# oneapi-src/ishmem

Hardware: AMD Instinct MI355X
Metric: GiB/s device-resident float32 sum-reduce at 1/2/4/8 PEs vs HBM+xGMI roofline (higher is better)
Workload: dtype f32; 1 GPU; float32 sum-reduce, 1024 MiB per PE, 1 PE(s), symmetric-heap device buffers; nreduce=268435456, bytes_per_pe=1073741824, pes=1, parallelism=1 PE self-reduce

## Files before the change

include/ishmem_capi.h:

```cpp
#ifndef ISHMEM_AMD_CAPI_H
#define ISHMEM_AMD_CAPI_H

#include <stddef.h>
#include <stdint.h>

#ifdef __cplusplus
extern "C" {
#endif

typedef enum {
    ISHMEMI_OP_AND = 0,
    ISHMEMI_OP_OR = 1,
    ISHMEMI_OP_XOR = 2,
    ISHMEMI_OP_MAX = 3,
    ISHMEMI_OP_MIN = 4,
    ISHMEMI_OP_SUM = 5,
    ISHMEMI_OP_PROD = 6,
    ISHMEMI_OP_COUNT = 7
} ishmemi_c_op_t;

typedef enum {
    ISHMEMI_DT_INT8 = 0,
    ISHMEMI_DT_INT16 = 1,
    ISHMEMI_DT_INT32 = 2,
// ... 198 lines not shown
    ISHMEMI_C_PATH_PHASED = 4,
    ISHMEMI_C_PATH_PERSISTENT = 5,
    ISHMEMI_C_PATH_ELEM = 6,
    ISHMEMI_C_PATH_STAGED = 7,
    ISHMEMI_C_PATH_COUNT = 8
} ishmemi_c_path_t;
const char *ishmemi_c_last_error(void);
int ishmemi_c_set_param(const char *name, long long value);
long long ishmemi_c_get_param(const char *name);
int ishmemi_c_phase_times(float *ms5);
int ishmemi_c_error_count(void);
size_t ishmemi_c_dtype_size(int dtype);
int ishmemi_c_op_dtype_valid(int op, int dtype);
int ishmemi_c_chunk_bounds(uint64_t nitems, int npes, int c, uint64_t *begin, uint64_t *end);
int ishmemi_c_path_limits(int npes, int colocated, long long *ll_limit, long long *fold_limit);
int ishmemi_c_bootstrap_selftest(int pe, int npes, const char *key, int value, int *out);
const char *ishmemi_c_version(void);

#ifdef __cplusplus
}
#endif

#endif
```

ishmem_amd/__init__.py:

```python
from __future__ import annotations

import ctypes
import sys

from ._lib import LIB_PATH, load

_L = load()

OPS = {"and": 0, "or": 1, "xor": 2, "max": 3, "min": 4, "sum": 5, "prod": 6}
DTYPES = {"int8": 0, "int16": 1, "int32": 2, "int64": 3, "uint8": 4, "uint16": 5,
          "uint32": 6, "uint64": 7, "float": 8, "double": 9,
          "half": 16, "bfloat16": 17}
ISHMEM_TEAM_INVALID = -1
ISHMEM_TEAM_WORLD = 0
ISHMEM_TEAM_SHARED = 1
ISHMEMX_TEAM_NODE = 2

TYPENAMES = {
    "char": "int8", "schar": "int8", "short": "int16", "int": "int32", "long": "int64",
    "longlong": "int64", "ptrdiff": "int64", "uchar": "uint8", "ushort": "uint16",
    "uint": "uint32", "ulong": "uint64", "ulonglong": "uint64", "int8": "int8",
    "int16": "int16", "int32": "int32", "int64": "int64", "uint8": "uint8", "uint16": "uint16",
    "uint32": "uint32", "uint64": "uint64", "size": "uint64", "float": "float", "double": "double",
}
# ... 178 lines not shown
    return int(_L.ishmemi_c_get_param(name.encode()))


PATH_NAMES = ("none", "single", "granule", "fold", "phased", "persistent", "elem", "staged")


def last_path() -> str:
    return PATH_NAMES[get_param("last_path")]


def path_limits(npes: int, colocated: bool) -> tuple[int, int]:
    ll, fold = ctypes.c_longlong(0), ctypes.c_longlong(0)
    if _L.ishmemi_c_path_limits(npes, int(bool(colocated)), ctypes.byref(ll), ctypes.byref(fold)):
        raise ValueError(f"path_limits: {last_error()}")
    return ll.value, fold.value


def reduce(op: str, dtype: str, dest: int, source: int, nreduce: int, team: int = ISHMEM_TEAM_WORLD) -> int:
    return _L.ishmemi_c_reduce(team, OPS[op], DTYPES[dtype], dest, source, nreduce)


def _event_handle(e) -> int | None:
    return getattr(e, "h", e) or None


def reduce_on_stream(op: str, dtype: str, dest: int, source: int, nreduce: int, ret: int | None,
                     stream: int, team: int = ISHMEM_TEAM_WORLD, deps=(), done=None) -> int:
    if deps or done is not None:
        hs = [_event_handle(e) for e in deps]
        arr = (ctypes.c_void_p * len(hs))(*hs) if hs else None
# ... 550 lines not shown
```

ishmem_amd/_lib.py:

```python
from __future__ import annotations

import ctypes
import os
from pathlib import Path

LIB_PATH = Path(__file__).resolve().parent / "libishmem_amd.so"
_VARIANT = os.environ.get("ISHMEM_AMD_LIB")

_vp, _i, _sz, _ll, _u64 = ctypes.c_void_p, ctypes.c_int, ctypes.c_size_t, ctypes.c_longlong, ctypes.c_uint64
_pd = ctypes.c_ssize_t
PROTOTYPES = [
    ("ishmemi_c_init", _i, []),
    ("ishmemi_c_init_pe", _i, [_i, _i, _i, ctypes.c_char_p]),
    ("ishmemi_c_launch_info", _i, [ctypes.POINTER(_i), ctypes.POINTER(_i), ctypes.POINTER(_i), ctypes.c_char_p, _sz,
                                   ctypes.c_char_p, _sz]),
    ("ishmemi_c_finalize", _i, []),
    ("ishmemi_c_initialized", _i, []),
    ("ishmemi_c_my_pe", _i, []),
    ("ishmemi_c_n_pes", _i, []),
    ("ishmemi_c_device", _i, []),
    ("ishmemi_c_init_thread", _i, [_i, ctypes.POINTER(_i)]),
    ("ishmemi_c_query_thread", _i, [ctypes.POINTER(_i)]),
    ("ishmemi_c_malloc", _vp, [_sz]),
    ("ishmemi_c_align", _vp, [_sz, _sz]),
# ... 63 lines not shown
    ("ishmemi_c_scan", _i, [_i, _i, _i, _vp, _vp, _sz]),
    ("ishmemi_c_scan_on_stream", _i, [_i, _i, _i, _vp, _vp, _sz, _vp, _vp]),
    ("ishmemi_c_broadcast", _i, [_i, _vp, _vp, _sz, _i]),
    ("ishmemi_c_broadcast_on_stream", _i, [_i, _vp, _vp, _sz, _i, _vp, _vp]),
    ("ishmemi_c_device_ctx", _vp, []),
    ("ishmemi_c_register_device_ctx_slot", _i, [_vp]),
    ("ishmemi_c_last_error", ctypes.c_char_p, []),
    ("ishmemi_c_set_param", _i, [ctypes.c_char_p, _ll]),
    ("ishmemi_c_get_param", _ll, [ctypes.c_char_p]),
    ("ishmemi_c_phase_times", _i, [ctypes.POINTER(ctypes.c_float)]),
    ("ishmemi_c_error_count", _i, []),
    ("ishmemi_c_dtype_size", _sz, [_i]),
    ("ishmemi_c_op_dtype_valid", _i, [_i, _i]),
    ("ishmemi_c_chunk_bounds", _i, [_u64, _i, _i, ctypes.POINTER(_u64), ctypes.POINTER(_u64)]),
    ("ishmemi_c_path_limits", _i, [_i, _i, ctypes.POINTER(_ll), ctypes.POINTER(_ll)]),
    ("ishmemi_c_bootstrap_selftest", _i, [_i, _i, ctypes.c_char_p, _i, ctypes.POINTER(_i)]),
    ("ishmemi_c_version", ctypes.c_char_p, []),
]

_lib = None


def load(build_if_missing: bool = True) -> ctypes.CDLL:
    global _lib
    if _lib is not None:
        return _lib
    if _VARIANT:
        lib = ctypes.CDLL(str(Path(_VARIANT).resolve()), mode=ctypes.RTLD_GLOBAL)
        for name, res, args in PROTOTYPES:
            fn = getattr(lib, name)
# ... 36 lines not shown
```

ishmem_amd/csrc/kernels.h:

```cpp
#pragma once
#include <hip/hip_runtime.h>
#include <stddef.h>
#include <stdint.h>

#include "types.h"

namespace ishmemi {

constexpr int kMaxPes = 16;
constexpr int kMaxBlocks = 1024;
constexpr int kPhases = 4;
constexpr int kPhaseStart = 0, kPhaseMid = 1, kPhaseEnd = 2, kPhaseSync = 3;
constexpr size_t kFlagWordsPerTeam = (size_t) kPhases * kMaxBlocks * kMaxPes;
constexpr size_t kTeamFlagBytes = kFlagWordsPerTeam * 4 + 256;
constexpr int kBlock = 256;
constexpr int kUnroll = 4;
constexpr int kFaninBlock = 64;
constexpr int kFaninMaxGrid = (int) ((1ull << 31) / kFaninBlock);

constexpr int kEpWords = 16;
constexpr int kLineWords = 16;
constexpr int kEpReplicas = 64;
constexpr int kEpRepLine = 1, kEpShardLine = kEpRepLine + kEpReplicas, kEpShards = 8;
constexpr int kEpTopLine = kEpShardLine + kEpShards;
// ... 113 lines not shown
#endif
constexpr int kRsRealignBlock = ISHMEMI_RS_REALIGN_BLOCK;
#ifndef ISHMEMI_REALIGN_PEEL
#define ISHMEMI_REALIGN_PEEL 256
#endif
constexpr uint64_t kRealignPeel = ISHMEMI_REALIGN_PEEL;

struct FaninArgs {
    const char *src[kMaxFanin];
    char *dst;
    uint64_t head, nitems, tail;
    int nsrc;
    int realign;
    uint32_t shift[kMaxFanin];
    uint64_t total;
};

struct PhaseArgs {
    const char *src[kMaxPes];
    const char *dstp[kMaxPes];
    char *dst;
    uint64_t head, nitems, tail;
    uint64_t items_per_chunk;
    uint32_t elem;
    int p, me;
    int peer_nt;
    uint32_t shift;
    uint64_t total;
    int whole;
    int xcd_group;
// ... 121 lines not shown
```

ishmem_amd/csrc/kernels_impl.h:

```cpp
#pragma once
#include <algorithm>
#include <map>
#include <mutex>
#include <type_traits>

#include "kernels.h"

namespace ishmemi {
namespace {

constexpr int kSysCoherent = 17;
constexpr int kNonTemporal = 2;
constexpr uint64_t kTile = (uint64_t) kBlock * kUnroll;
#ifndef ISHMEMI_AR_OCC
#define ISHMEMI_AR_OCC 4
#endif


template <typename T>
struct alignas(16) Vec {
    T e[16 / sizeof(T)];
};

template <typename T>
// ... 711 lines not shown

template <typename I>
__device__ __forceinline__ I nt_load(const I *p)
{
    if constexpr (sizeof(I) == 16) return __builtin_bit_cast(I, __builtin_nontemporal_load((const u32x4 *) p));
    else if constexpr (is_fp16_v<I>) return I{__builtin_nontemporal_load((const uint16_t *) p)};
    else return __builtin_nontemporal_load(p);
}

template <typename T, int OP, bool VEC, int NS>
__global__ __launch_bounds__(kFaninBlock) void fanin_kernel(FaninArgs a)
{
    using Item = std::conditional_t<VEC, Vec<T>, T>;
    constexpr uint64_t IB = sizeof(Item);
    const uint64_t head_bytes = VEC ? a.head * sizeof(T) : 0;
    const uint64_t stride = (uint64_t) gridDim.x * kFaninBlock;
    for (uint64_t i = (uint64_t) blockIdx.x * kFaninBlock + threadIdx.x; i < a.nitems; i += stride) {
        const uint64_t off = head_bytes + i * IB;
        Item acc;
        if constexpr (NS == 1) {
            acc = nt_load((const Item *) (a.src[0] + off));
        } else if constexpr (NS == 2 && VEC) {
            const uint64_t wo = off - (uint64_t) threadIdx.x * IB;
            const uint32_t lo = (uint32_t) (threadIdx.x * IB);
            const Item x0 = bload<Item>(make_rsrc(uniform_ptr(a.src[0] + wo)), lo);
            asm volatile("s_waitcnt vmcnt(0)" ::: "memory");
            const Item x1 = bload<Item>(make_rsrc(uniform_ptr(a.src[1] + wo)), lo);
            acc = op1<T, OP>(x0, x1);
        } else if constexpr (NS == 2) {
            const Item x0 = nt_load((const Item *) (a.src[0] + off));
            const Item x1 = nt_load((const Item *) (a.src[1] + off));
            acc = op1<T, OP>(x0, x1);
// ... 76 lines not shown
#pragma unroll
    for (int j = 0; j < NS; ++j) realign_issue<kNonTemporal>(a.src[j], a.shift[j], a.total, wo, edge[j], A[j], B[j]);
    __syncthreads();
    Vec<T> acc = __builtin_bit_cast(Vec<T>, realign_finish(edge[0], A[0], B[0], a.shift[0]));
    if constexpr (NS == 2)
        acc = op1<T, OP>(acc, __builtin_bit_cast(Vec<T>, realign_finish(edge[1], A[1], B[1], a.shift[1])));
    if (i0 + tid < a.nitems) wt_store(make_rsrc(uniform_ptr(a.dst + wo)), tid * 16u, acc);
}

template <typename T, int OP, int NS>
__global__ __launch_bounds__(kRealignBlock) void fanin_realign_kernel(FaninArgs a)
{
    static_assert(NS == 1 || NS == 2, "realigned fan-in: 1 or 2 sources");
    __shared__ u32x4 edge[NS][kRealignWaves + 1];
    const uint32_t tid = threadIdx.x;
    const uint64_t stride = (uint64_t) gridDim.x * kRealignBlock;
    const uint64_t first = (uint64_t) blockIdx.x * kRealignBlock;
    if (stride >= a.nitems) {
        if (first < a.nitems) fanin_realign_block<T, OP, NS>(a, edge, first);
    } else {
        for (uint64_t i0 = first; i0 < a.nitems; i0 += stride) {
            fanin_realign_block<T, OP, NS>(a, edge, i0);
            __syncthreads();
        }
    }
    if (blockIdx.x == 0) {
        const uint64_t tail_off = a.head + a.nitems * (16 / sizeof(T));
        for (int pass = 0; pass < 2; ++pass) {
            const uint64_t cnt = pass == 0 ? a.head : a.tail;
            for (uint64_t t = tid; t < cnt; t += kRealignBlock) {
                const uint64_t e = pass == 0 ? t : tail_off + t;
                T acc = ((const T *) a.src[0])[e];
                if constexpr (NS == 2) acc = op1<T, OP>(acc, ((const T *) a.src[1])[e]);
                ((T *) a.dst)[e] = acc;
            }
        }
    }
// ... 619 lines not shown
```

ishmem_amd/csrc/runtime.cpp:

```cpp
#include <hip/hip_runtime.h>
#include <stdio.h>
#include <stdlib.h>
#include <string.h>
#include <strings.h>
#include <stdint.h>
#include <errno.h>
#include <sys/prctl.h>
#include <unistd.h>

#include <algorithm>
#include <chrono>
#include <limits>
#include <map>
#include <mutex>
#include <string>
#include <vector>

#include "bootstrap.h"
#include "kernels.h"
#include "types.h"

namespace ishmemi {
namespace {

// ... 152 lines not shown
    return s && *s && (strcmp(s, "0") == 0 || strcasecmp(s, "false") == 0);
}
bool env_flag_true(const char *name)
{
    const char *s = getenv(name);
    return s && *s && !env_flag_false(name);
}

void warn_unknown_env()
{
    static const char *const known[] = {
        "DEBUG", "ENABLE_VERBOSE_PRINT", "STACK_PRINT_LIMIT", "ENABLE_GPU_IPC", "ENABLE_GPU_IPC_PIDFD",
        "SYMMETRIC_SIZE", "ENABLE_ACCESSIBLE_HOST_HEAP", "NBI_COUNT", "MWAIT_BURST", "SHMEM_LIB_NAME",
        "MPI_LIB_NAME", "PMI_LIB_NAME", "TEAMS_MAX", "TEAM_SHARED_ONLY_SELF", "RUNTIME", "RUNTIME_USE_OSHMPI", "ROOT",
        "PE", "NPES", "DEVICE", "BOOTSTRAP_KEY", "TIMEOUT_MS", "MAX_BLOCKS", "WAIT_SLOTS", "LL_MAX_BYTES",
        "ONESHOT_P2_MAX_BYTES", "PHASED_MIN_BYTES", "PHASED_PEER_NT", "STAGING_SIZE", "STAGING_SLOTS",
        "STAGED_COPY_KERNEL", "STREAM_ORDER", "FLAGS_KIND", "EP_UNCACHED", "BARRIER_KIND", "XGMI_LL_MAX_BYTES",
        "XGMI_FOLD_MAX_BYTES", "PUT_SIGNAL_FUSED_MAX_BYTES", "TEST_FLAGS_UNAVAILABLE", "TEST_PCI_BUS",
        "AMD_LIB", "OFFLOAD_ARCH", "BENCH_SAME_DEVICE", "BENCH_EMULATE_SHARE1", "BENCH_SETUP_WATCHDOG_S"};
    for (char **e = ::environ; e && *e; ++e) {
        if (strncmp(*e, "ISHMEM_", 7) != 0) continue;
        const char *name = *e + 7, *eq = strchr(name, '=');
        const size_t len = eq ? (size_t) (eq - name) : strlen(name);
        bool ok = false;
        for (const char *k : known) ok = ok || (strlen(k) == len && strncmp(k, name, len) == 0);
        if (!ok) fprintf(stderr, "[ishmem_amd] WARN: Environment variable 'ISHMEM_%.*s' is not a supported variable\n", (int) len, name);
    }
}

long long wait_slots_floor() { return std::max<long long>(1, env_ll("GPU_MAX_HW_QUEUES", 4)); }

// ... 7 lines not shown

struct TeamMem {
    uint32_t *flags[kMaxPes] = {};
    uint64_t *ring[kMaxPes] = {};
    int pool_idx = -1;
    char *fold_scratch = nullptr;
    size_t fold_scratch_bytes = 0;
};

struct PoolBlock {
    uint32_t *ptr = nullptr;
    hipIpcMemHandle_t handle{};
    bool in_use = false;
};

constexpr long long kPhasedOff = std::numeric_limits<long long>::max();
constexpr long long kPhasedDefault = 4ll << 20;

struct PeRecord {
    int32_t pe, pid, device, flags_kind;
    int32_t flags_kind_requested;
    char pci_bus[32];
    uint64_t heap_size;
    int64_t max_blocks, ll_max_bytes, oneshot_p2, phased_min;
    uint64_t staging_bytes;
    int64_t staging_slots;
    int64_t xgmi_ll_max, xgmi_fold_max;
    hipIpcMemHandle_t heap_handle;
    hipIpcMemHandle_t flags_handle;
};
// ... 50 lines not shown
    hipStream_t last_stream = nullptr;
    bool last_stream_set = false;
    bool stream_order = false;
    long long oneshot_p2 = 32ll << 20;
    long long phased_min = kPhasedDefault;
    hipEvent_t order_ev = nullptr;
    hipEvent_t staging_ev = nullptr;
    bool staging_used = false;
    int staging_slots = kStagingSlotsDefault;
    int staged_copy_kernel = 0;
    bool test_flags_unavailable = false;
    int phased_peer_nt = 0;
    int ar_shifted = 1;
    int rs_xcd = 1;
    int last_path = ISHMEMI_C_PATH_NONE;
    int direct_p2 = 1;
    int direct_max_pes = 4;
    int direct_inplace = 1;
    long long xgmi_ll_max = -1, xgmi_fold_max = -1;
    double xgmi_link_bps = 76.8e9;
    hipEvent_t ev_in[kMaxStagingSlots] = {}, ev_red[kMaxStagingSlots] = {}, ev_out[kMaxStagingSlots] = {};

    Team teams[kMaxTeams];
    int max_blocks = kMaxBlocks;
    long long ll_max_bytes = (long long) kLLDefaultBytes;
    long long timeout_ms = 60000;
    int debug = 0;
    int error_count = 0;
    uint64_t *trace = nullptr;
    bool phase_events = false, phase_recorded = false;
// ... 265 lines not shown
    const uintptr_t d = (uintptr_t) dst;
    bool ok = !pl.vec && nsrc >= 1 && nsrc <= 2 && n * es >= kRealignMinBytes && d % es == 0;
    for (int j = 0; ok && j < nsrc; ++j) ok = (uintptr_t) srcs[j] % es == 0;
    if (!ok) return;
    const uint64_t h = std::min<uint64_t>(n, ((kRealignPeel - d % kRealignPeel) % kRealignPeel) / es);
    f.head = h;
    f.nitems = (n - h) * es / 16;
    f.tail = n - h - f.nitems * (16 / es);
    for (int j = 0; j < nsrc; ++j) f.shift[j] = (uint32_t) (((uintptr_t) srcs[j] + h * es) % 16);
    f.total = n * es;
    f.realign = 1;
    pl.grid = (int) std::max<uint64_t>(1, std::min<uint64_t>((f.nitems + kRealignBlock - 1) / kRealignBlock,
                                                             (uint64_t) kRealignMaxGrid));
}

int launch_copy(void *dst, const void *src, size_t bytes, hipStream_t st)
{
    if (bytes == 0 || dst == src) return 0;
    FaninArgs f{};
    f.src[0] = (const char *) src;
    f.dst = (char *) dst;
    f.nsrc = 1;
    const void *srcs[1] = {src};
    Plan pl;
    plan_fanin(f, pl, dst, srcs, 1, bytes, 1);
    HIP_TRY(launch_fanin(ISHMEMI_OP_OR, ISHMEMI_DT_UINT8, pl.vec, f, pl.grid, st));
    return 0;
}

constexpr double kHopUs = 1.0;
constexpr long long kUnlimited = std::numeric_limits<long long>::max();
struct Line {
    double a_us, b_us_per_byte;
};
Line model_ll(int p, double L) { return {4.5 + 0.5 * (p - 2) + 1 * kHopUs, 2e6 / L}; }
Line model_fold(int p, double L) { return {9.0 + 0.75 * (p - 2) + 2 * kHopUs, 1e6 / L}; }
Line model_rsag(int p, double L) { return {9.5 + 2.5 * (p - 2) + 3 * kHopUs, 2e6 / (p * L)}; }

long long crossover(const Line &f, const Line &g)
{
// ... 240 lines not shown
        if (mark(0)) return 1;
        if (team_barrier(a, st)) return 1;
        if (mark(1)) return 1;
        HIP_TRY(launch_rs_phase(op, dt, ph, st));
        if (mark(2)) return 1;
        if (!direct) {
            if (team_barrier(a, st)) return 1;
            if (mark(3)) return 1;
            HIP_TRY(launch_ag_phase(ph, st));
        } else if (mark(3)) {
            return 1;
        }
        if (mark(4)) return 1;
        if (team_barrier(a, st)) return 1;
        if (mark(5)) return 1;
        if (inplace_fold && launch_copy(dst, scratch, nb, st)) return 1;
        s.phase_recorded = s.phase_recorded || ev;
        return 0;
    }
    if (t.size == 2 && (long long) nb <= lim.oneshot && disjoint) {
        a.oneshot = 1;
        a.items_per_chunk = pl.nitems;
        a.seg_items = seg_items(pl.nitems);
        pl.grid = (int) std::max<uint64_t>(
            1, std::min<uint64_t>(nsegs(pl.nitems, a.seg_items), (uint64_t) s.max_blocks));
    }
    s.last_path = ISHMEMI_C_PATH_PERSISTENT;
    HIP_TRY(launch_allreduce(op, dt, pl.vec, a, pl.grid, st));
    return 0;
}

// ... 75 lines not shown
            HIP_TRY(hipEventCreateWithFlags(&s.ev_in[i], hipEventDisableTiming));
            HIP_TRY(hipEventCreateWithFlags(&s.ev_red[i], hipEventDisableTiming));
            HIP_TRY(hipEventCreateWithFlags(&s.ev_out[i], hipEventDisableTiming));
        }
    }
    if (staging_acquire(s, st)) return 1;
    HIP_TRY(hipEventRecord(s.ev_red[0], st));
    HIP_TRY(hipStreamWaitEvent(s.copy_in, s.ev_red[0], 0));
    bool used[kMaxStagingSlots] = {};
    for (size_t off = 0, k = 0; off < n; off += chunk, ++k) {
        const int sl = (int) (k % (size_t) nslots);
        char *buf = s.staging + (size_t) sl * slot_bytes;
        const size_t m = std::min(chunk, n - off);
        if (used[sl]) HIP_TRY(hipStreamWaitEvent(s.copy_in, s.ev_out[sl], 0));
        if (src_dev) {
            if (launch_copy(buf, src_dev + off * es, m * es, s.copy_in)) return 1;
        } else {
            HIP_TRY(hipMemcpyAsync(buf, (const char *) src + off * es, m * es, hipMemcpyDefault, s.copy_in));
        }
        HIP_TRY(hipEventRecord(s.ev_in[sl], s.copy_in));
        HIP_TRY(hipStreamWaitEvent(st, s.ev_in[sl], 0));
        if (s.teams[team].size > 1) {
            const bool ll = ll_eligible(s, s.teams[team], buf, buf, m * es);
            if (ll ? reduce_ll(s, team, op, dt, buf, buf, m * es, ret, st)
                   : reduce_heap(s, team, op, dt, buf, buf, m, ret, st))
                return 1;
        }
        HIP_TRY(hipEventRecord(s.ev_red[sl], st));
        HIP_TRY(hipStreamWaitEvent(s.copy_out, s.ev_red[sl], 0));
        if (dst_dev) {
            if (launch_copy(dst_dev + off * es, buf, m * es, s.copy_out)) return 1;
        } else {
            HIP_TRY(hipMemcpyAsync((char *) dst + off * es, buf, m * es, hipMemcpyDefault, s.copy_out));
        }
        HIP_TRY(hipEventRecord(s.ev_out[sl], s.copy_out));
        used[sl] = true;
    }
    for (int sl = 0; sl < nslots; ++sl)
        if (used[sl]) HIP_TRY(hipStreamWaitEvent(st, s.ev_out[sl], 0));
    return staging_release(s, st);
}

int team_sync_locked(State &s, int team, hipStream_t st, int *ret);

template <typename A>
int fill_team_sync_args(State &s, int team, A &a, std::string &why)
// ... 74 lines not shown
        if (collect_launch(s, team, dst, s.staging, segb, ret, st, segoff)) return 1;
    }
    s.last_path = ISHMEMI_C_PATH_STAGED;
    return staging_release(s, st);
}

int collect_on_stream_impl(int team, void *dst, const void *src, size_t nbytes, int *ret, hipStream_t st)
{
    State &s = S();
    std::lock_guard<std::mutex> lk(s.mu);
    if (team_call(s, "collect", team)) return 1;
    Team &t = s.teams[team];
    if (ret) HIP_TRY(hipMemsetAsync(ret, 0, sizeof(int), st));
    if (t.size == 1) {
        s.last_path = ISHMEMI_C_PATH_SINGLE;
        if (nbytes && dst != src && launch_copy(dst, src, nbytes, st)) return 1;
        return mark_stream(s, st);
    }
    if (!in_heap(s, dst)) return fail("collect: dest must be symmetric-heap memory");
    if (!in_heap(s, src)) return fail("collect: source must be symmetric-heap memory");
    if (order_stream(s, st)) return 1;
    CollectArgs a;
    memset(&a, 0, sizeof(a));
    std::string why;
    if (fill_team_sync_args(s, team, a, why)) return fail("collect: " + why);
    char *slot = s.count_slots + (size_t) team * 64;
    for (int j = 0; j < t.size; ++j) {
        const int gpe = t.start + j * t.stride;
        a.src[j] = translate(s, src, gpe);
        a.count_at[j] = (const uint64_t *) translate(s, slot, gpe);
        if (!a.src[j] || !a.count_at[j]) return fail("collect: buffer not mapped for PE " + std::to_string(gpe));
// ... 8 lines not shown
    s.last_path = ISHMEMI_C_PATH_PERSISTENT;
    HIP_TRY(launch_collect_dyn(a, grid, st));
    return mark_stream(s, st);
}

int fcollect_impl(int team, void *dst, const void *src, size_t nbytes, int *ret, hipStream_t st,
                  bool blocking, int staged = -1)
{
    State &s = S();
    std::lock_guard<std::mutex> lk(s.mu);
    if (team_call(s, "fcollect", team)) return 1;
    Team &t = s.teams[team];
    if (ret) HIP_TRY(hipMemsetAsync(ret, 0, sizeof(int), st));
    if (t.size == 1) {
        s.last_path = ISHMEMI_C_PATH_SINGLE;
        if (nbytes && dst != src && launch_copy(dst, src, nbytes, st)) return 1;
    } else {
        if (staged < 0 && !device_writable(s, dst)) return fail("fcollect: dest must be heap, device or pinned host memory");
        uint64_t nb[kMaxPes];
        for (int j = 0; j < t.size; ++j) nb[j] = nbytes;
        if (staged < 0) staged = in_heap(s, src) ? 0 : 1;
        if (nbytes == 0) {
            s.last_path = ISHMEMI_C_PATH_NONE;
            if (team_sync_locked(s, team, st, ret)) return 1;
        } else if (!staged && ll_eligible(s, t, dst, src, nbytes) && 2 * nbytes <= ll_capacity(t.size)) {
            s.last_path = ISHMEMI_C_PATH_GRANULE;
            if (reduce_ll(s, team, ISHMEMI_OP_OR, ISHMEMI_DT_UINT8, dst, src, nbytes, ret, st, kLLCollect)) return 1;
        } else if (staged) {
            if (order_stream(s, st) || collect_staged(s, team, (char *) dst, (const char *) src, nb, ret, st)) return 1;
        } else if (collect_launch(s, team, dst, src, nb, ret, st)) {
            return 1;
// ... 54 lines not shown
int alltoall_impl(int team, void *dst, const void *src, size_t nbytes, int *ret, hipStream_t st, bool blocking,
                  bool checked)
{
    State &s = S();
    std::lock_guard<std::mutex> lk(s.mu);
    if (team_call(s, "alltoall", team)) return 1;
    Team &t = s.teams[team];
    if (nbytes > 0 && (!dst || !src)) return fail("alltoall: null buffer");
    if (t.size > 1 && nbytes > 0 && !checked) {
        const uint64_t e = alltoall_arg_errors(s, t, dst, src, nbytes);
        if (e) return fail(alltoall_arg_message(e));
    }
    if (ret) HIP_TRY(hipMemsetAsync(ret, 0, sizeof(int), st));
    if (t.size == 1) {
        s.last_path = ISHMEMI_C_PATH_SINGLE;
        if (nbytes && dst != src && launch_copy(dst, src, nbytes, st)) return 1;
    } else if (nbytes == 0) {
        s.last_path = ISHMEMI_C_PATH_NONE;
        if (team_sync_locked(s, team, st, ret)) return 1;
    } else if (ll_eligible(s, t, dst, src, nbytes) && 2 * nbytes <= ll_capacity(t.size)) {
        s.last_path = ISHMEMI_C_PATH_GRANULE;
        if (reduce_ll(s, team, ISHMEMI_OP_OR, ISHMEMI_DT_UINT8, dst, src, nbytes, ret, st, kLLAlltoall)) return 1;
    } else {
        uint64_t nb[kMaxPes], off[kMaxPes];
        const char *srcs[kMaxPes];
        for (int j = 0; j < t.size; ++j) {
            const char *pj = translate(s, src, t.start + j * t.stride);
            if (!pj) return fail("alltoall: source not mapped for PE " + std::to_string(t.start + j * t.stride));
            srcs[j] = pj + (uint64_t) t.my_idx * nbytes;
            off[j] = (uint64_t) j * nbytes;
            nb[j] = nbytes;
// ... 78 lines not shown
{
    State &s = S();
    std::lock_guard<std::mutex> lk(s.mu);
    if (team_call(s, "reduce_scatter", team)) return 1;
    Team &t = s.teams[team];
    if (!op_dtype_valid(op, dt)) return fail("reduce_scatter: invalid (op, dtype) pair");
    if (n > 0 && (!dst || !src)) return fail("reduce_scatter: null buffer");
    if (n > 0 && !checked) {
        const uint64_t e = reduce_scatter_arg_errors(s, t, op, dt, dst, src, n);
        if (e) return fail(reduce_scatter_arg_message(e));
    }
    const size_t B = n * dtype_size(dt);
    if (ret) HIP_TRY(hipMemsetAsync(ret, 0, sizeof(int), st));
    if (t.size == 1) {
        s.last_path = ISHMEMI_C_PATH_SINGLE;
        if (B && launch_copy(device_view(s, dst), src, B, st)) return 1;
    } else if (n == 0) {
        s.last_path = ISHMEMI_C_PATH_NONE;
        if (team_sync_locked(s, team, st, ret)) return 1;
    } else if (ll_eligible(s, t, dst, src, B) && B <= ll_capacity(t.size)) {
        s.last_path = ISHMEMI_C_PATH_GRANULE;
        if (reduce_ll(s, team, op, dt, device_view(s, dst), src, B, ret, st, kLLReduceScatter)) return 1;
    } else if (reduce_scatter_heap(s, team, op, dt, device_view(s, dst), src, n, ret, st)) {
        return 1;
    }
    return finish_call(s, team, st, blocking);
}

enum RmaKind { kRmaBlocking = 0, kRmaNbi = 1, kRmaOnStream = 2 };

int check_pe(const State &s, const std::string &what, int pe)
// ... 648 lines not shown
    return staging_release(s, st);
}

int scan_impl(int team, int dt, int inclusive, void *dst, const void *src, size_t n, int *ret,
              hipStream_t st, bool blocking)
{
    State &s = S();
    std::lock_guard<std::mutex> lk(s.mu);
    if (s.initialized && !scan_dtype_valid(dt)) return fail("scan: invalid dtype");
    if (team_call(s, "scan", team)) return 1;
    Team &t = s.teams[team];
    const size_t es = dtype_size(dt);
    if (ret) HIP_TRY(hipMemsetAsync(ret, 0, sizeof(int), st));
    if (t.size == 1) {
        s.last_path = ISHMEMI_C_PATH_SINGLE;
        if (n && inclusive && dst != src && launch_copy(dst, src, n * es, st)) return 1;
        if (n && !inclusive) HIP_TRY(hipMemsetAsync(dst, 0, n * es, st));
    } else if (n == 0) {
        s.last_path = ISHMEMI_C_PATH_NONE;
        if (team_sync_locked(s, team, st, ret)) return 1;
    } else {
        if (!in_heap(s, dst) || !in_heap(s, src)) return fail("scan: buffers must be symmetric-heap memory");
        if (((uintptr_t) dst | (uintptr_t) src) % es) return fail("scan: misaligned buffers");
        const uint64_t ipc_max = ((s.staging_bytes / es) / (uint64_t) t.size) & ~uint64_t(63);
        const uint64_t seg = ipc_max * (uint64_t) t.size;
        const uintptr_t d0 = (uintptr_t) dst, s0 = (uintptr_t) src, nb = n * es;
        const bool disjoint = d0 + nb <= s0 || s0 + nb <= d0;
        if (ll_eligible(s, t, dst, src, nb)) {
            s.last_path = ISHMEMI_C_PATH_GRANULE;
            if (reduce_ll(s, team, ISHMEMI_OP_SUM, dt, dst, src, nb, ret, st, inclusive ? kLLInscan : kLLExscan))
                return 1;
// ... 45 lines not shown
    if (!valid_team(s, team)) return fail("reduce: invalid team handle");
    Team &t = s.teams[team];
    if (t.my_idx < 0) return fail("reduce: calling PE is not a member of the team");
    if (n > 0 && (!dst || !src)) return fail("reduce: null buffer");
    const size_t es = dtype_size(dt);
    const size_t bytes = n * es;
    if (ret) HIP_TRY(hipMemsetAsync(ret, 0, sizeof(int), st));
    PtrInfo di, si;

    if (t.size == 1) {
        s.last_path = ISHMEMI_C_PATH_SINGLE;
        if (n > 0 && dst != src) {
            const Kind kd = ptr_info(s, dst, di).kind(), ks = ptr_info(s, src, si).kind();
            if (kd == Kind::Host || ks == Kind::Host) {
                if (reduce_staged(s, team, op, dt, dst, src, n, ret, st, di, si)) return 1;
            } else if (launch_copy(dst, src, bytes, st)) {
                return 1;
            }
        }
    } else if (n == 0) {
        s.last_path = ISHMEMI_C_PATH_NONE;
        if (team_sync_locked(s, team, st, ret)) return 1;
    } else if (ll_eligible(s, t, dst, src, bytes) && ptr_info(s, dst, di).kind() != Kind::Host &&
               ptr_info(s, src, si).kind() != Kind::Host) {
        s.last_path = ISHMEMI_C_PATH_GRANULE;
        if (reduce_ll(s, team, op, dt, dst, src, bytes, ret, st)) return 1;
    } else if (in_heap(s, dst) && in_heap(s, src)) {
        if (reduce_heap(s, team, op, dt, dst, src, n, ret, st)) return 1;
    } else {
        if (reduce_staged(s, team, op, dt, dst, src, n, ret, st, di, si)) return 1;
    }
// ... 137 lines not shown
                      "IPC-mapped heaps; there is no proxy path)";
    if (env_flag_true("ISHMEM_ENABLE_ACCESSIBLE_HOST_HEAP") && g_env_error.empty())
        g_env_error = std::string("ISHMEM_ENABLE_ACCESSIBLE_HOST_HEAP=") + getenv("ISHMEM_ENABLE_ACCESSIBLE_HOST_HEAP") +
                      " is not supported: the symmetric heap is device memory shared over IPC (host buffers "
                      "are accepted by every call and staged)";
    s.max_blocks = (int) std::min<long long>(kMaxBlocks, std::max<long long>(1, env_ll("ISHMEM_MAX_BLOCKS", kMaxBlocks)));
    s.timeout_ms = std::max<long long>(1, env_ll("ISHMEM_TIMEOUT_MS", 60000));
    s.ll_max_bytes = std::min<long long>((long long) kLLMaxBytes,
                                         std::max<long long>(0, env_bytes("ISHMEM_LL_MAX_BYTES", (long long) kLLDefaultBytes)));
    s.debug = debug_level();
    s.trace = nullptr;
    s.stream_order = env_ll("ISHMEM_STREAM_ORDER", 0) != 0;
    s.oneshot_p2 = std::max<long long>(0, env_bytes("ISHMEM_ONESHOT_P2_MAX_BYTES", 32ll << 20));
    s.phased_min = env_bytes("ISHMEM_PHASED_MIN_BYTES", kPhasedDefault);
    if (s.phased_min < 0) s.phased_min = kPhasedOff;
    s.staging_bytes = (env_size("ISHMEM_STAGING_SIZE", (size_t) 128 << 20) + kHeapAlign - 1) &
                      ~(size_t) (kHeapAlign - 1);
    s.staging_slots = (int) std::min<long long>(kMaxStagingSlots, std::max<long long>(2, env_ll("ISHMEM_STAGING_SLOTS", kStagingSlotsDefault)));
    s.staged_copy_kernel = (int) (env_ll("ISHMEM_STAGED_COPY_KERNEL", kStagedCopyKernelDefault) & 3);
    const size_t heap_request = env_size("ISHMEM_SYMMETRIC_SIZE", (size_t) 4 << 30);
    const int first_kind = (int) std::min<long long>(kFlagsCoarse, std::max<long long>(0, env_ll("ISHMEM_FLAGS_KIND", 0)));
#ifdef ISHMEMI_TEST_HOOKS
    s.test_flags_unavailable = env_ll("ISHMEM_TEST_FLAGS_UNAVAILABLE", 0) != 0;
#else
    for (const char *hook : {"ISHMEM_TEST_FLAGS_UNAVAILABLE", "ISHMEM_TEST_PCI_BUS"})
        if (getenv(hook) && g_env_error.empty())
            g_env_error = std::string(hook) + " is a test hook, honoured only by libishmem_amd_testhooks.so";
#endif
    const bool ep_uncached = env_ll("ISHMEM_EP_UNCACHED", 0) != 0;
    s.phased_peer_nt = env_ll("ISHMEM_PHASED_PEER_NT", 0) != 0;
// ... 1251 lines not shown
                      void *stream)
{
    if (!op_dtype_valid(op, dtype)) return fail("combine: invalid (op, dtype) pair");
    if (nsrc < 1 || nsrc > kMaxFanin) return fail("combine: nsrc must be 1..16");
    if (n == 0) return 0;
    if (!dst || !srcs) return fail("combine: null pointer");
    FaninArgs f{};
    for (int i = 0; i < nsrc; ++i) {
        if (!srcs[i]) return fail("combine: null source");
        f.src[i] = (const char *) srcs[i];
    }
    f.dst = (char *) dst;
    f.nsrc = nsrc;
    Plan pl;
    plan_fanin(f, pl, dst, srcs, nsrc, n, dtype_size(dtype));
    HIP_TRY(launch_fanin(op, dtype, pl.vec, f, pl.grid, (hipStream_t) stream));
    return 0;
}

int ishmemi_c_pull_probe(void *dst, const void *const *srcs, int nsrc, size_t nbytes, int policy,
                         void *stream)
{
    if (nsrc < 1 || nsrc > kMaxFanin) return fail("pull_probe: nsrc must be 1..16");
    if (!dst || !srcs || nbytes % 16 || ((uintptr_t) dst & 15))
        return fail("pull_probe: 16-B aligned pointers and a multiple of 16 bytes required");
    if (nbytes == 0) return 0;
    FaninArgs f{};
    for (int i = 0; i < nsrc; ++i) {
        if (!srcs[i] || ((uintptr_t) srcs[i] & 15)) return fail("pull_probe: misaligned or null source");
        f.src[i] = (const char *) srcs[i];
// ... 152 lines not shown

int ishmemi_c_broadcast_on_stream(int team, void *dest, const void *source, size_t nbytes, int root,
                                  int *ret, void *stream)
{
    State &s = S();
    std::lock_guard<std::mutex> lk(s.mu);
    if (!member_call(s, team)) return fail("broadcast_on_stream: not initialized, invalid team or caller not a member");
    const Team &t = s.teams[team];
    if (root < 0 || root >= t.size) return fail("broadcast_on_stream: root is not a team index");
    hipStream_t st = (hipStream_t) stream;
    if (ret) HIP_TRY(hipMemsetAsync(ret, 0, sizeof(int), st));
    if (t.size == 1) {
        s.last_path = ISHMEMI_C_PATH_SINGLE;
        if (nbytes && dest != source) {
            if (device_writable(s, dest) && classify(s, source) != Kind::Host) {
                if (launch_copy(dest, source, nbytes, st)) return 1;
            } else {
                HIP_TRY(hipMemcpyAsync(dest, source, nbytes, hipMemcpyDefault, st));
            }
        }
        return mark_stream(s, st);
    }
    if (nbytes == 0) {
        s.last_path = ISHMEMI_C_PATH_NONE;
        return team_sync_locked(s, team, st, ret) || mark_stream(s, st);
    }
    if (!in_heap(s, source)) return fail("broadcast_on_stream: source must be symmetric-heap memory");
    if (!device_writable(s, dest)) return fail("broadcast_on_stream: dest must be heap, device or pinned host memory");
    if (ll_eligible(s, t, dest, source, nbytes) && 2 * nbytes <= ll_capacity(t.size)) {
        s.last_path = ISHMEMI_C_PATH_GRANULE;
        if (reduce_ll(s, team, ISHMEMI_OP_OR, ISHMEMI_DT_UINT8, dest, source, nbytes, ret, st, kLLBroadcast, root)) return 1;
// ... 79 lines not shown
    State &s = S();
    std::lock_guard<std::mutex> lk(s.mu);
    const std::string n = name ? name : "";
    if (n == "max_blocks") s.max_blocks = (int) std::min<long long>(kMaxBlocks, std::max<long long>(1, value));
    else if (n == "staged_copy_kernel") s.staged_copy_kernel = (int) (value & 3);
    else if (n == "wait_slots") {
        if (value < wait_slots_floor())
            return fail("set_param: wait_slots " + std::to_string(value) + " is below " +
                        std::to_string(wait_slots_floor()) + " (GPU_MAX_HW_QUEUES), see ISHMEM_WAIT_SLOTS");
        set_wait_slots((int) std::min<long long>(1 << 20, value));
    }
    else if (n == "timeout_ms") s.timeout_ms = std::max<long long>(1, value);
    else if (n == "stream_order") s.stream_order = value != 0;
    else if (n == "oneshot_p2_max_bytes") s.oneshot_p2 = std::max<long long>(0, value);
    else if (n == "phased_min_bytes") s.phased_min = value < 0 ? kPhasedOff : value;
    else if (n == "ll_max_bytes") s.ll_max_bytes = std::min<long long>((long long) kLLMaxBytes, std::max<long long>(0, value));
    else if (n == "put_signal_fused_max_bytes") s.put_signal_fused_max = std::max<long long>(0, value);
    else if (n == "debug") s.debug = (int) value;
    else if (n == "phased_peer_nt") s.phased_peer_nt = value != 0;
    else if (n == "xgmi_ll_max_bytes") s.xgmi_ll_max = std::max<long long>(-1, value);
    else if (n == "xgmi_fold_max_bytes") s.xgmi_fold_max = std::max<long long>(-1, value);
    else if (n == "xgmi_link_mbps") {
        if (value <= 0) return fail("set_param: xgmi_link_mbps must be positive");
        s.xgmi_link_bps = (double) value * 1e6;
    }
    else if (n == "realign_grid_cap") set_realign_grid_cap((int) std::min<long long>(std::max<long long>(value, 0), 1 << 30));
    else if (n == "collect_realign") set_collect_realign((int) (value != 0));
    else if (n == "ar_shifted") s.ar_shifted = value != 0;
    else if (n == "rs_xcd") s.rs_xcd = value != 0;
    else if (n == "direct_p2") s.direct_p2 = value != 0;
// ... 32 lines not shown
    if (n == "xgmi_fold_max_bytes") return s.xgmi_fold_max;
    if (n == "xgmi_link_mbps") return (long long) (s.xgmi_link_bps / 1e6);
    if (n == "teams_max") return s.teams_max;
    if (n == "flag_block_bytes") return s.initialized ? (long long) (kBaseAllocBytes + s.team_block_bytes) : 0;
    if (n == "flag_block_pool_bytes") return (long long) (s.team_pool.size() * kTeamAllocBytes);
    if (n == "flag_block_bytes_round5") return (long long) kRound5FlagBytes;
    for (int k = 0; k < 8; ++k)
        if (n == std::string("init_us_") + kInitPhase[k]) return (long long) s.init_us[k];
    if (n == "debug") return s.debug;
    if (n == "phased_peer_nt") return s.phased_peer_nt;
    if (n == "realign_grid_cap") return realign_grid_cap();
    if (n == "collect_realign") return collect_realign();
    if (n == "ar_shifted") return s.ar_shifted;
    if (n == "rs_xcd") return s.rs_xcd;
    if (n == "last_path") return s.last_path;
    if (n == "direct_p2") return s.direct_p2;
    if (n == "direct_inplace") return s.direct_inplace;
    if (n == "block_spin") return s.block_spin;
    if (n == "direct_max_pes") return s.direct_max_pes;
    if (n == "phase_unaligned") return phase_unaligned();
    if (n == "flags_fine_grained") return s.flags_kind != kFlagsCoarse ? 1 : 0;
    if (n == "flags_kind") return s.flags_kind;
    if (n == "staging_bytes") return (long long) s.staging_bytes;
    if (n == "staging_slots") return s.staging_slots;
    if (n == "heap_bytes") return (long long) s.heap_size;
    if (n == "device_share") return device_share();
    if (n == "launch_words") return (long long) (uintptr_t) s.kern_ep;
    if (n == "cu_count") {
        int dev = 0, cus = 0;
        if (hipGetDevice(&dev) != hipSuccess ||
// ... 31 lines not shown
    *end = std::min<uint64_t>(*begin + ipc, nitems);
    return 0;
}

int ishmemi_c_path_limits(int npes, int colocated, long long *ll_limit, long long *fold_limit)
{
    if (npes < 1 || npes > kMaxPes || !ll_limit || !fold_limit) return fail("path_limits: invalid arguments");
    State &s = S();
    std::lock_guard<std::mutex> lk(s.mu);
    const PathLimits r = path_limits(s, npes, colocated != 0);
    *ll_limit = r.ll;
    *fold_limit = r.fold;
    return 0;
}

int ishmemi_c_bootstrap_selftest(int pe, int npes, const char *key, int value, int *out)
{
    ShmBootstrap b;
    std::string err;
    if (b.attach(pe, npes, key ? key : "selftest", 20000, err)) return fail(err);
    if (b.allgather(&value, out, sizeof(int), err)) return fail(err);
    if (b.barrier(err)) return fail(err);
    return 0;
}

const char *ishmemi_c_version(void) { return "ishmem_amd 0.1.0 (reduction path; ref ishmem 1.5.1)"; }

}
```

Baseline: 3147 GiB/s.

## Alternate fan-in traversal direction across calls to reuse cache-resident tails

Adds a per-stream record of the address ranges the last large fan-in or copy touched. When the next launch overlaps those ranges, the grid walks its blocks in the opposite direction, so the region touched last by the previous pass is read first while it may still sit in the last-level cache. The feature is on by default for payloads of at least 512 MiB and is skipped under graph capture and for in-place overlap. The kernels index blocks through a reversible mapping, and a new C API, Python wrapper and tunable parameters expose the choice. The benefit relies on consecutive calls touching the same buffers.

```diff
diff --git a/include/ishmem_capi.h b/include/ishmem_capi.h
--- a/include/ishmem_capi.h
+++ b/include/ishmem_capi.h
@@ -236,6 +236,14 @@
 int ishmemi_c_op_dtype_valid(int op, int dtype);
 int ishmemi_c_chunk_bounds(uint64_t nitems, int npes, int c, uint64_t *begin, uint64_t *end);
 int ishmemi_c_path_limits(int npes, int colocated, long long *ll_limit, long long *fold_limit);
+#define ISHMEMI_C_FANIN_RANGES 17
+typedef struct {
+    int32_t valid, order, nranges, reserved;
+    uint64_t stream;
+    uint64_t ranges[2 * ISHMEMI_C_FANIN_RANGES];
+} ishmemi_c_fanin_record_t;
+int ishmemi_c_fanin_order(ishmemi_c_fanin_record_t *rec, int mode, long long min_bytes, int capturing,
+                          const void *stream, const uint64_t *ranges, int nranges, uint64_t payload_bytes);
 int ishmemi_c_bootstrap_selftest(int pe, int npes, const char *key, int value, int *out);
 const char *ishmemi_c_version(void);
 
diff --git a/ishmem_amd/__init__.py b/ishmem_amd/__init__.py
--- a/ishmem_amd/__init__.py
+++ b/ishmem_amd/__init__.py
@@ -216,6 +216,24 @@
     if _L.ishmemi_c_path_limits(npes, int(bool(colocated)), ctypes.byref(ll), ctypes.byref(fold)):
         raise ValueError(f"path_limits: {last_error()}")
     return ll.value, fold.value
+
+
+class FaninOrder:
+
+    RANGES = 17
+
+    def __init__(self):
+        self.rec = (ctypes.c_uint64 * (3 + 2 * self.RANGES))()
+
+    def __call__(self, dest: int, sources, nbytes: int, stream: int = 0, mode: int = 0, min_bytes: int = 0,
+                 capturing: bool = False) -> int:
+        ops = [dest, *sources]
+        r = (ctypes.c_uint64 * (2 * len(ops)))(*[x for p in ops for x in (p, p + nbytes)])
+        o = _L.ishmemi_c_fanin_order(ctypes.addressof(self.rec), mode, min_bytes, int(capturing), stream or None,
+                                     r, len(ops), nbytes)
+        if o < 0:
+            raise ValueError("fanin_order: invalid arguments")
+        return o
 
 
 def reduce(op: str, dtype: str, dest: int, source: int, nreduce: int, team: int = ISHMEM_TEAM_WORLD) -> int:
diff --git a/ishmem_amd/_lib.py b/ishmem_amd/_lib.py
--- a/ishmem_amd/_lib.py
+++ b/ishmem_amd/_lib.py
@@ -101,6 +101,7 @@
     ("ishmemi_c_op_dtype_valid", _i, [_i, _i]),
     ("ishmemi_c_chunk_bounds", _i, [_u64, _i, _i, ctypes.POINTER(_u64), ctypes.POINTER(_u64)]),
     ("ishmemi_c_path_limits", _i, [_i, _i, ctypes.POINTER(_ll), ctypes.POINTER(_ll)]),
+    ("ishmemi_c_fanin_order", _i, [_vp, _i, _ll, _i, _vp, ctypes.POINTER(_u64), _i, _u64]),
     ("ishmemi_c_bootstrap_selftest", _i, [_i, _i, ctypes.c_char_p, _i, ctypes.POINTER(_i)]),
     ("ishmemi_c_version", ctypes.c_char_p, []),
 ]
diff --git a/ishmem_amd/csrc/kernels.h b/ishmem_amd/csrc/kernels.h
--- a/ishmem_amd/csrc/kernels.h
+++ b/ishmem_amd/csrc/kernels.h
@@ -151,6 +151,7 @@
     int realign;
     uint32_t shift[kMaxFanin];
     uint64_t total;
+    int reverse;
 };
 
 struct PhaseArgs {
diff --git a/ishmem_amd/csrc/kernels_impl.h b/ishmem_amd/csrc/kernels_impl.h
--- a/ishmem_amd/csrc/kernels_impl.h
+++ b/ishmem_amd/csrc/kernels_impl.h
@@ -749,8 +749,10 @@
     using Item = std::conditional_t<VEC, Vec<T>, T>;
     constexpr uint64_t IB = sizeof(Item);
     const uint64_t head_bytes = VEC ? a.head * sizeof(T) : 0;
-    const uint64_t stride = (uint64_t) gridDim.x * kFaninBlock;
-    for (uint64_t i = (uint64_t) blockIdx.x * kFaninBlock + threadIdx.x; i < a.nitems; i += stride) {
+    const uint64_t nblocks = (a.nitems + kFaninBlock - 1) / kFaninBlock;
+    for (uint64_t b = blockIdx.x; b < nblocks; b += gridDim.x) {
+        const uint64_t i = (a.reverse ? nblocks - 1 - b : b) * kFaninBlock + threadIdx.x;
+        if (i >= a.nitems) continue;
         const uint64_t off = head_bytes + i * IB;
         Item acc;
         if constexpr (NS == 1) {
@@ -857,13 +859,13 @@
     static_assert(NS == 1 || NS == 2, "realigned fan-in: 1 or 2 sources");
     __shared__ u32x4 edge[NS][kRealignWaves + 1];
     const uint32_t tid = threadIdx.x;
-    const uint64_t stride = (uint64_t) gridDim.x * kRealignBlock;
-    const uint64_t first = (uint64_t) blockIdx.x * kRealignBlock;
-    if (stride >= a.nitems) {
-        if (first < a.nitems) fanin_realign_block<T, OP, NS>(a, edge, first);
+    const uint64_t nblocks = (a.nitems + kRealignBlock - 1) / kRealignBlock;
+    auto first_item = [&](uint64_t b) { return (a.reverse ? nblocks - 1 - b : b) * kRealignBlock; };
+    if (gridDim.x >= nblocks) {
+        if (blockIdx.x < nblocks) fanin_realign_block<T, OP, NS>(a, edge, first_item(blockIdx.x));
     } else {
-        for (uint64_t i0 = first; i0 < a.nitems; i0 += stride) {
-            fanin_realign_block<T, OP, NS>(a, edge, i0);
+        for (uint64_t b = blockIdx.x; b < nblocks; b += gridDim.x) {
+            fanin_realign_block<T, OP, NS>(a, edge, first_item(b));
             __syncthreads();
         }
     }
diff --git a/ishmem_amd/csrc/runtime.cpp b/ishmem_amd/csrc/runtime.cpp
--- a/ishmem_amd/csrc/runtime.cpp
+++ b/ishmem_amd/csrc/runtime.cpp
@@ -190,7 +190,7 @@
         "SYMMETRIC_SIZE", "ENABLE_ACCESSIBLE_HOST_HEAP", "NBI_COUNT", "MWAIT_BURST", "SHMEM_LIB_NAME",
         "MPI_LIB_NAME", "PMI_LIB_NAME", "TEAMS_MAX", "TEAM_SHARED_ONLY_SELF", "RUNTIME", "RUNTIME_USE_OSHMPI", "ROOT",
         "PE", "NPES", "DEVICE", "BOOTSTRAP_KEY", "TIMEOUT_MS", "MAX_BLOCKS", "WAIT_SLOTS", "LL_MAX_BYTES",
-        "ONESHOT_P2_MAX_BYTES", "PHASED_MIN_BYTES", "PHASED_PEER_NT", "STAGING_SIZE", "STAGING_SLOTS",
+        "ONESHOT_P2_MAX_BYTES", "PHASED_MIN_BYTES", "FANIN_ORDER_MIN_BYTES", "PHASED_PEER_NT", "STAGING_SIZE", "STAGING_SLOTS",
         "STAGED_COPY_KERNEL", "STREAM_ORDER", "FLAGS_KIND", "EP_UNCACHED", "BARRIER_KIND", "XGMI_LL_MAX_BYTES",
         "XGMI_FOLD_MAX_BYTES", "PUT_SIGNAL_FUSED_MAX_BYTES", "TEST_FLAGS_UNAVAILABLE", "TEST_PCI_BUS",
         "AMD_LIB", "OFFLOAD_ARCH", "BENCH_SAME_DEVICE", "BENCH_EMULATE_SHARE1", "BENCH_SETUP_WATCHDOG_S"};
@@ -228,6 +228,7 @@
     bool in_use = false;
 };
 
+constexpr long long kFaninOrderMinDefault = 512ll << 20;
 constexpr long long kPhasedOff = std::numeric_limits<long long>::max();
 constexpr long long kPhasedDefault = 4ll << 20;
 
@@ -308,6 +309,10 @@
     int ar_shifted = 1;
     int rs_xcd = 1;
     int last_path = ISHMEMI_C_PATH_NONE;
+    int fanin_order_mode = 0;
+    long long fanin_order_min = kFaninOrderMinDefault;
+    ishmemi_c_fanin_record_t fanin_rec = {};
+    int last_fanin_order = 0;
     int direct_p2 = 1;
     int direct_max_pes = 4;
     int direct_inplace = 1;
@@ -603,7 +608,55 @@
                                                              (uint64_t) kRealignMaxGrid));
 }
 
-int launch_copy(void *dst, const void *src, size_t bytes, hipStream_t st)
+using FaninRecord = ishmemi_c_fanin_record_t;
+
+bool ranges_overlap(uint64_t a0, uint64_t a1, uint64_t b0, uint64_t b1) { return a0 < b1 && b0 < a1; }
+
+int fanin_order(FaninRecord &rec, int mode, long long min_bytes, bool capture, const void *stream,
+                const uint64_t *ranges, int nranges, uint64_t payload_bytes)
+{
+    nranges = std::max(1, std::min(nranges, ISHMEMI_C_FANIN_RANGES));
+    bool self_overlap = false;
+    for (int j = 1; j < nranges; ++j)
+        self_overlap = self_overlap || ranges_overlap(ranges[0], ranges[1], ranges[2 * j], ranges[2 * j + 1]);
+    const bool exempt = capture || (long long) std::min<uint64_t>(payload_bytes, INT64_MAX) < min_bytes || self_overlap;
+    if (mode == 0 && exempt) return 0;
+    int order = mode == 2 ? 1 : 0;
+    if (mode == 0 && rec.valid && rec.stream == (uint64_t) (uintptr_t) stream) {
+        bool hit = false;
+        for (int i = 0; i < rec.nranges && !hit; ++i)
+            for (int j = 0; j < nranges && !hit; ++j)
+                hit = ranges_overlap(rec.ranges[2 * i], rec.ranges[2 * i + 1], ranges[2 * j], ranges[2 * j + 1]);
+        if (hit) order = !rec.order;
+    }
+    if (exempt) return order;
+    rec.valid = 1;
+    rec.order = order;
+    rec.stream = (uint64_t) (uintptr_t) stream;
+    rec.nranges = nranges;
+    memcpy(rec.ranges, ranges, sizeof(uint64_t) * 2 * (size_t) nranges);
+    return order;
+}
+
+bool capturing(hipStream_t st);
+
+int choose_fanin_order(State &s, const void *dst, const void *const *srcs, int nsrc, size_t bytes, hipStream_t st)
+{
+    uint64_t r[2 * ISHMEMI_C_FANIN_RANGES];
+    r[0] = (uint64_t) (uintptr_t) dst;
+    r[1] = r[0] + bytes;
+    for (int j = 0; j < nsrc; ++j) {
+        r[2 * j + 2] = (uint64_t) (uintptr_t) srcs[j];
+        r[2 * j + 3] = r[2 * j + 2] + bytes;
+    }
+    const bool cap = s.fanin_order_mode == 0 && (long long) bytes >= s.fanin_order_min && capturing(st);
+    s.last_fanin_order = fanin_order(s.fanin_rec, s.fanin_order_mode, s.fanin_order_min, cap, st, r, nsrc + 1, bytes);
+    return s.last_fanin_order;
+}
+
+enum class CopyOrder { kForward, kChoose };
+
+int launch_copy(void *dst, const void *src, size_t bytes, hipStream_t st, CopyOrder whose)
 {
     if (bytes == 0 || dst == src) return 0;
     FaninArgs f{};
@@ -613,6 +666,7 @@
     const void *srcs[1] = {src};
     Plan pl;
     plan_fanin(f, pl, dst, srcs, 1, bytes, 1);
+    f.reverse = whose == CopyOrder::kChoose ? choose_fanin_order(S(), dst, srcs, 1, bytes, st) : 0;
     HIP_TRY(launch_fanin(ISHMEMI_OP_OR, ISHMEMI_DT_UINT8, pl.vec, f, pl.grid, st));
     return 0;
 }
@@ -883,7 +937,7 @@
         if (mark(4)) return 1;
         if (team_barrier(a, st)) return 1;
         if (mark(5)) return 1;
-        if (inplace_fold && launch_copy(dst, scratch, nb, st)) return 1;
+        if (inplace_fold && launch_copy(dst, scratch, nb, st, CopyOrder::kForward)) return 1;
         s.phase_recorded = s.phase_recorded || ev;
         return 0;
     }
@@ -989,7 +1043,7 @@
         const size_t m = std::min(chunk, n - off);
         if (used[sl]) HIP_TRY(hipStreamWaitEvent(s.copy_in, s.ev_out[sl], 0));
         if (src_dev) {
-            if (launch_copy(buf, src_dev + off * es, m * es, s.copy_in)) return 1;
+            if (launch_copy(buf, src_dev + off * es, m * es, s.copy_in, CopyOrder::kForward)) return 1;
         } else {
             HIP_TRY(hipMemcpyAsync(buf, (const char *) src + off * es, m * es, hipMemcpyDefault, s.copy_in));
         }
@@ -1004,7 +1058,7 @@
         HIP_TRY(hipEventRecord(s.ev_red[sl], st));
         HIP_TRY(hipStreamWaitEvent(s.copy_out, s.ev_red[sl], 0));
         if (dst_dev) {
-            if (launch_copy(dst_dev + off * es, buf, m * es, s.copy_out)) return 1;
+            if (launch_copy(dst_dev + off * es, buf, m * es, s.copy_out, CopyOrder::kForward)) return 1;
         } else {
             HIP_TRY(hipMemcpyAsync((char *) dst + off * es, buf, m * es, hipMemcpyDefault, s.copy_out));
         }
@@ -1109,7 +1163,7 @@
     if (ret) HIP_TRY(hipMemsetAsync(ret, 0, sizeof(int), st));
     if (t.size == 1) {
         s.last_path = ISHMEMI_C_PATH_SINGLE;
-        if (nbytes && dst != src && launch_copy(dst, src, nbytes, st)) return 1;
+        if (nbytes && dst != src && launch_copy(dst, src, nbytes, st, CopyOrder::kChoose)) return 1;
         return mark_stream(s, st);
     }
     if (!in_heap(s, dst)) return fail("collect: dest must be symmetric-heap memory");
@@ -1148,7 +1202,7 @@
     if (ret) HIP_TRY(hipMemsetAsync(ret, 0, sizeof(int), st));
     if (t.size == 1) {
         s.last_path = ISHMEMI_C_PATH_SINGLE;
-        if (nbytes && dst != src && launch_copy(dst, src, nbytes, st)) return 1;
+        if (nbytes && dst != src && launch_copy(dst, src, nbytes, st, CopyOrder::kChoose)) return 1;
     } else {
         if (staged < 0 && !device_writable(s, dst)) return fail("fcollect: dest must be heap, device or pinned host memory");
         uint64_t nb[kMaxPes];
@@ -1233,7 +1287,7 @@
     if (ret) HIP_TRY(hipMemsetAsync(ret, 0, sizeof(int), st));
     if (t.size == 1) {
         s.last_path = ISHMEMI_C_PATH_SINGLE;
-        if (nbytes && dst != src && launch_copy(dst, src, nbytes, st)) return 1;
+        if (nbytes && dst != src && launch_copy(dst, src, nbytes, st, CopyOrder::kChoose)) return 1;
     } else if (nbytes == 0) {
         s.last_path = ISHMEMI_C_PATH_NONE;
         if (team_sync_locked(s, team, st, ret)) return 1;
@@ -1342,7 +1396,7 @@
     if (ret) HIP_TRY(hipMemsetAsync(ret, 0, sizeof(int), st));
     if (t.size == 1) {
         s.last_path = ISHMEMI_C_PATH_SINGLE;
-        if (B && launch_copy(device_view(s, dst), src, B, st)) return 1;
+        if (B && launch_copy(device_view(s, dst), src, B, st, CopyOrder::kForward)) return 1;
     } else if (n == 0) {
         s.last_path = ISHMEMI_C_PATH_NONE;
         if (team_sync_locked(s, team, st, ret)) return 1;
@@ -2021,7 +2075,7 @@
     if (ret) HIP_TRY(hipMemsetAsync(ret, 0, sizeof(int), st));
     if (t.size == 1) {
         s.last_path = ISHMEMI_C_PATH_SINGLE;
-        if (n && inclusive && dst != src && launch_copy(dst, src, n * es, st)) return 1;
+        if (n && inclusive && dst != src && launch_copy(dst, src, n * es, st, CopyOrder::kChoose)) return 1;
         if (n && !inclusive) HIP_TRY(hipMemsetAsync(dst, 0, n * es, st));
     } else if (n == 0) {
         s.last_path = ISHMEMI_C_PATH_NONE;
@@ -2097,7 +2151,7 @@
             const Kind kd = ptr_info(s, dst, di).kind(), ks = ptr_info(s, src, si).kind();
             if (kd == Kind::Host || ks == Kind::Host) {
                 if (reduce_staged(s, team, op, dt, dst, src, n, ret, st, di, si)) return 1;
-            } else if (launch_copy(dst, src, bytes, st)) {
+            } else if (launch_copy(dst, src, bytes, st, CopyOrder::kChoose)) {
                 return 1;
             }
         }
@@ -2265,6 +2319,8 @@
     s.oneshot_p2 = std::max<long long>(0, env_bytes("ISHMEM_ONESHOT_P2_MAX_BYTES", 32ll << 20));
     s.phased_min = env_bytes("ISHMEM_PHASED_MIN_BYTES", kPhasedDefault);
     if (s.phased_min < 0) s.phased_min = kPhasedOff;
+    s.fanin_order_min = std::max<long long>(0, env_bytes("ISHMEM_FANIN_ORDER_MIN_BYTES", kFaninOrderMinDefault));
+    s.fanin_rec = {};
     s.staging_bytes = (env_size("ISHMEM_STAGING_SIZE", (size_t) 128 << 20) + kHeapAlign - 1) &
                       ~(size_t) (kHeapAlign - 1);
     s.staging_slots = (int) std::min<long long>(kMaxStagingSlots, std::max<long long>(2, env_ll("ISHMEM_STAGING_SLOTS", kStagingSlotsDefault)));
@@ -3546,6 +3602,9 @@
     f.nsrc = nsrc;
     Plan pl;
     plan_fanin(f, pl, dst, srcs, nsrc, n, dtype_size(dtype));
+    State &s = S();
+    std::lock_guard<std::mutex> lk(s.mu);
+    f.reverse = choose_fanin_order(s, dst, srcs, nsrc, n * dtype_size(dtype), (hipStream_t) stream);
     HIP_TRY(launch_fanin(op, dtype, pl.vec, f, pl.grid, (hipStream_t) stream));
     return 0;
 }
@@ -3728,7 +3787,7 @@
         s.last_path = ISHMEMI_C_PATH_SINGLE;
         if (nbytes && dest != source) {
             if (device_writable(s, dest) && classify(s, source) != Kind::Host) {
-                if (launch_copy(dest, source, nbytes, st)) return 1;
+                if (launch_copy(dest, source, nbytes, st, CopyOrder::kChoose)) return 1;
             } else {
                 HIP_TRY(hipMemcpyAsync(dest, source, nbytes, hipMemcpyDefault, st));
             }
@@ -3838,6 +3897,11 @@
     else if (n == "stream_order") s.stream_order = value != 0;
     else if (n == "oneshot_p2_max_bytes") s.oneshot_p2 = std::max<long long>(0, value);
     else if (n == "phased_min_bytes") s.phased_min = value < 0 ? kPhasedOff : value;
+    else if (n == "fanin_order") {
+        if (value < 0 || value > 2) return fail("set_param: fanin_order is 0 (automatic), 1 (forward) or 2 (reverse)");
+        s.fanin_order_mode = (int) value;
+    }
+    else if (n == "fanin_order_min_bytes") s.fanin_order_min = std::max<long long>(0, value);
     else if (n == "ll_max_bytes") s.ll_max_bytes = std::min<long long>((long long) kLLMaxBytes, std::max<long long>(0, value));
     else if (n == "put_signal_fused_max_bytes") s.put_signal_fused_max = std::max<long long>(0, value);
     else if (n == "debug") s.debug = (int) value;
@@ -3900,6 +3964,9 @@
     if (n == "ar_shifted") return s.ar_shifted;
     if (n == "rs_xcd") return s.rs_xcd;
     if (n == "last_path") return s.last_path;
+    if (n == "fanin_order") return s.fanin_order_mode;
+    if (n == "fanin_order_min_bytes") return s.fanin_order_min;
+    if (n == "last_fanin_order") return s.last_fanin_order;
     if (n == "direct_p2") return s.direct_p2;
     if (n == "direct_inplace") return s.direct_inplace;
     if (n == "block_spin") return s.block_spin;
@@ -3961,6 +4028,13 @@
     return 0;
 }
 
+int ishmemi_c_fanin_order(ishmemi_c_fanin_record_t *rec, int mode, long long min_bytes, int capture,
+                          const void *stream, const uint64_t *ranges, int nranges, uint64_t payload_bytes)
+{
+    if (!rec || !ranges || nranges < 1 || nranges > ISHMEMI_C_FANIN_RANGES || mode < 0 || mode > 2) return -1;
+    return fanin_order(*rec, mode, min_bytes, capture != 0, stream, ranges, nranges, payload_bytes);
+}
+
 int ishmemi_c_bootstrap_selftest(int pe, int npes, const char *key, int value, int *out)
 {
     ShmBootstrap b;
```

Result: faster. 3199 GiB/s, median of 6 (+1.6%).
